# jakubbober/discrete-curvature-rewiring

Hardware: AMD Instinct MI355X
Metric: SDRF iterations/sec (higher is better)
Workload: dtype f64; 1 GPU; S100k: preferential-attachment graph N=100000 m=10 E=999900 (PCG64 seed 12345), Balanced Forman curvature, full recompute every iteration, remove_edges=True, tau=163.0, removal_bound=0.95; parallelism=single GPU

## Files before the change

### discrete-curvature-rewiring_amd/csrc/dcr_sdrf.hip

```cpp
#include <cstdlib>
#include "dcr_internal.h"
#include <cstdio>

namespace dcr {

struct RowView {
    const int2 *rowinfo;
    const int32_t *col;
    const int32_t *slot_row;
};

__device__ __host__ inline double bfc_formula(int d1, int d2, int T, int s1, int s2, int gamma) {
    int dmax = d1 > d2 ? d1 : d2, dmin = d1 < d2 ? d1 : d2;
    double r = 2.0 / (double)d1;
    r = r + 2.0 / (double)d2;
    r = r - 2.0;
    r = r + (double)(2 * (int64_t)T) / (double)dmax;
    r = r + (double)T / (double)dmin;
    if (s1 == 0 || s2 == 0) return r;
    double q = 1.0 / (double)gamma;
    q = q / (double)dmax;
    q = q * (double)(s1 + s2);
    return r + q;
}
// ... 21 lines not shown
            cv[q] = ok[q] ? curv[s] : 0.0;
        }
#pragma unroll
        for (int q = 0; q < 4; ++q) ru[q] = ok[q] ? g.rowinfo[u[q]] : make_int2(0, 0);
#pragma unroll
        for (int q = 0; q < 4; ++q) {
            const int64_t s = s0 + q * stride;
            if (!ok[q] || (int)(s - ru[q].x) >= ru[q].y || v[q] <= u[q]) continue;
            body((int)s, u[q], v[q], cv[q], acc...);
        }
    }
}

__global__ void __launch_bounds__(256) k_argext_edges(RowView g, int64_t cap_total, const double *curv, int want_max,
                                                       int excl_u, int excl_v, const DevResult *res, Ext *partial) {
    __shared__ double shv[4];
    __shared__ int shs[4];
    if (excl_u == -2) {
        excl_u = res->cand_i;
        excl_v = res->cand_j;
    }
    double best_v = 0.0;
    int best_s = -1;
    walk_edge_slots(
        g, cap_total, curv,
        [=](int s, int u, int v, double cv, double &bv, int &bs) {
            if (u == excl_u && v == excl_v) return;
            ext_take(bv, bs, cv, s, want_max);
        },
        best_v, best_s);
    ext_block_reduce(best_v, best_s, want_max, shv, shs);
    if (threadIdx.x == 0) partial[blockIdx.x] = ext_make(best_v, best_s);
}

__global__ void __launch_bounds__(256) k_argext_edges_both(RowView g, int64_t cap_total, const double *curv, Ext *part_min, Ext *part_max,
                                                            unsigned *clear_words, int64_t n_clear_words, DevResult *res) {
    __shared__ double shv[4];
    __shared__ int shs[4];
    for (int64_t i = (int64_t)blockIdx.x * blockDim.x + threadIdx.x; i < n_clear_words; i += (int64_t)gridDim.x * blockDim.x) clear_words[i] = 0u;
    if (n_clear_words > 0 && blockIdx.x == 0 && threadIdx.x == 0) res->touched_n = 0;
    double lo_v = 0.0, hi_v = 0.0;
    int lo_s = -1, hi_s = -1;
    walk_edge_slots(
        g, cap_total, curv,
        [](int s, int, int, double cv, double &lv, int &ls, double &hv, int &hs) {
            ext_take(lv, ls, cv, s, 0);
            ext_take(hv, hs, cv, s, 1);
        },
        lo_v, lo_s, hi_v, hi_s);
    ext_block_reduce(lo_v, lo_s, 0, shv, shs);
    if (threadIdx.x == 0) part_min[blockIdx.x] = ext_make(lo_v, lo_s);
    __syncthreads();
    ext_block_reduce(hi_v, hi_s, 1, shv, shs);
    if (threadIdx.x == 0) part_max[blockIdx.x] = ext_make(hi_v, hi_s);
}

__device__ inline void reduce_partials(const Ext *partial, int nparts, int want_max, double &best_v, int &best_s) {
    __shared__ double shv[16];
    __shared__ int shs[16];
    best_v = 0.0;
    best_s = -1;
    for (int i = threadIdx.x; i < nparts; i += blockDim.x) {
        const Ext e = partial[i];
        ext_take(best_v, best_s, e.val, e.slot, want_max);
    }
    ext_block_reduce(best_v, best_s, want_max, shv, shs);
}

__device__ inline void argext_final_body(const RowView &g, const Ext *partial, int nparts, int want_max, DevResult *res) {
    double best_v;
    int best_s;
    reduce_partials(partial, nparts, want_max, best_v, best_s);
    if (threadIdx.x == 0) {
        res->ext_val = best_v;
        res->ext_slot = best_s;
        const int eu = best_s >= 0 ? g.slot_row[best_s] : -1, ev = best_s >= 0 ? g.col[best_s] : -1;
        res->ext_u = eu;
        res->ext_v = ev;
        res->ext_du = best_s >= 0 ? g.rowinfo[eu].y : 0;
        res->ext_dv = best_s >= 0 ? g.rowinfo[ev].y : 0;
    }
}

__global__ void __launch_bounds__(1024) k_argext_final(RowView g, const Ext *partial, int nparts, int want_max,
                                                        DevResult *res) {
    argext_final_body(g, partial, nparts, want_max, res);
}

__global__ void __launch_bounds__(256) k_argmax_array(const double *a, int64_t n, const DevResult *res, Ext *partial) {
    __shared__ double shv[4];
    __shared__ int shs[4];
    if (res) n = res->n_cand;
    double best_v = 0.0;
    int best_s = -1;
    for (int64_t i = (int64_t)blockIdx.x * blockDim.x + threadIdx.x; i < n; i += (int64_t)gridDim.x * blockDim.x) {
        ext_take(best_v, best_s, a[i], (int)i, 1);
    }
    ext_block_reduce(best_v, best_s, 1, shv, shs);
    if (threadIdx.x == 0) partial[blockIdx.x] = ext_make(best_v, best_s);
}

__global__ void __launch_bounds__(256) k_argmax_final(const Ext *partial, int nparts, DevResult *res) {
    double best_v;
    int best_s;
    reduce_partials(partial, nparts, 1, best_v, best_s);
    if (threadIdx.x == 0) res->imp_argmax = best_s;
}

__device__ inline void store_candidate(DevResult *res, const int32_t *ci, const int32_t *cj, int64_t idx) {
    const int32_t a = ci[idx], b = cj[idx];
    res->cand_i = a < b ? a : b;
    res->cand_j = a < b ? b : a;
}

constexpr unsigned T_EMPTY = 0xFFFFFFFFu;

__device__ inline unsigned g_hash(unsigned key, unsigned mask) { return (key * 0x9E3779B1u >> 7) & mask; }

__device__ inline int g_find(const int32_t *keys, unsigned mask, int key) {
    unsigned h = g_hash((unsigned)key, mask);
    while (true) {
        const int e = keys[h];
        if (e == key) return (int)h;
        if ((unsigned)e == T_EMPTY) return -1;
        h = (h + 1) & mask;
    }
}

__device__ inline void g_find4(const int32_t *keys, unsigned mask, const int (&key)[4], const bool (&valid)[4], int (&out)[4]) {
    unsigned h[4];
    int e[4];
#pragma unroll
    for (int q = 0; q < 4; ++q) {
        h[q] = g_hash((unsigned)key[q], mask);
        e[q] = valid[q] ? keys[h[q]] : (int)T_EMPTY;
    }
#pragma unroll
    for (int q = 0; q < 4; ++q) {
        out[q] = -1;
        if (!valid[q]) continue;
        while (true) {
            if (e[q] == key[q]) { out[q] = (int)h[q]; break; }
            if ((unsigned)e[q] == T_EMPTY) break;
            h[q] = (h[q] + 1) & mask;
            e[q] = keys[h[q]];
        }
    }
}

struct ImpBuf {
    int32_t *keys, *posx, *posy;
    int32_t *c1, *c2;
    int32_t *clsx, *clsy;
    double *impb, *impc;
    int32_t *rowcount, *rowoff;
    uint32_t *adjbits;
    ImpStats *st;
};

__global__ void __launch_bounds__(256) k_imp_insert(RowView g, ImpBuf B, int x, int y, unsigned mask, const Ext *amax_parts, int amax_n,
                                                     DevResult *res) {
    const int nblocks = (int)gridDim.x - (amax_parts ? 1 : 0);
    if ((int)blockIdx.x == nblocks) {
        argext_final_body(g, amax_parts, amax_n, 1, res);
        return;
    }
    const int2 rx = g.rowinfo[x], ry = g.rowinfo[y];
    const int total = rx.y + ry.y;
    for (int t = blockIdx.x * blockDim.x + threadIdx.x; t < total; t += nblocks * blockDim.x) {
        const bool isx = t < rx.y;
        const int p = isx ? t : t - rx.y;
        const int k = g.col[(isx ? rx.x : ry.x) + p];
        if (isx) {
            B.c1[p] = 0;
            B.clsx[p] = k == y ? 2 : 0;
        } else {
            B.c2[p] = 0;
            B.clsy[p] = k == x ? 2 : 0;
            if (k == x) B.st->pos_x_in_y = p;
        }
        if (k == (isx ? y : x)) continue;
        unsigned h = g_hash((unsigned)k, mask);
        while (true) {
            const unsigned old = atomicCAS((unsigned *)&B.keys[h], T_EMPTY, (unsigned)k);
            if (old == T_EMPTY || old == (unsigned)k) break;
            h = (h + 1) & mask;
        }
        if (isx) B.posx[h] = p;
        else B.posy[h] = p;
    }
    if (blockIdx.x == 0 && threadIdx.x == 0) {
        B.st->x = x;
        B.st->y = y;
        B.st->dx = rx.y;
        B.st->dy = ry.y;
        B.st->table_mask = (int)mask;
        B.st->T = 0;
        B.st->deg_min_is_one = (rx.y < ry.y ? rx.y : ry.y) == 1;
        B.st->done_rows = 0;
        B.st->done_draw = 0;
    }
}

__global__ void __launch_bounds__(256) k_imp_clear(ImpBuf B, int64_t ts) {
    const int64_t tid = (int64_t)blockIdx.x * blockDim.x + threadIdx.x, nth = (int64_t)gridDim.x * blockDim.x;
    for (int64_t i = tid; i < ts; i += nth) {
        B.keys[i] = -1;
        B.posx[i] = -1;
        B.posy[i] = -1;
    }
    if (tid == 0) B.st->pos_x_in_y = -1;
}

struct Mx {
    int m, c, s;
};

__device__ inline Mx mx_join(Mx a, Mx b) {
    Mx r;
    if (a.m == b.m) {
        r.m = a.m;
        r.c = a.c + b.c;
        r.s = a.s > b.s ? a.s : b.s;
    } else if (a.m > b.m) {
        r.m = a.m;
        r.c = a.c;
        r.s = a.s > b.m ? a.s : b.m;
    } else {
        r.m = b.m;
        r.c = b.c;
        r.s = b.s > a.m ? b.s : a.m;
    }
    return r;
}

__device__ inline Mx mx_add(Mx a, int v) {
    Mx b;
    b.m = v;
    b.c = 1;
    b.s = -1;
    return mx_join(a, b);
}

__device__ inline void block_stats(const int32_t *c, int n, int *cnt_pos, Mx *mx, int *shi) {
    int pos = 0;
    Mx m;
    m.m = -1;
    m.c = 0;
    m.s = -1;
    for (int i = threadIdx.x; i < n; i += blockDim.x) {
        const int v = c[i];
        pos += v > 0;
        m = mx_add(m, v);
    }
    for (int off = 32; off > 0; off >>= 1) {
        pos += __shfl_xor(pos, off);
        Mx o;
        o.m = __shfl_xor(m.m, off);
        o.c = __shfl_xor(m.c, off);
        o.s = __shfl_xor(m.s, off);
        m = mx_join(m, o);
    }
    const int lane = threadIdx.x & 63, wid = threadIdx.x >> 6, nw = blockDim.x >> 6;
    __syncthreads();
    if (lane == 0) {
        shi[wid * 4 + 0] = pos;
        shi[wid * 4 + 1] = m.m;
        shi[wid * 4 + 2] = m.c;
        shi[wid * 4 + 3] = m.s;
    }
    __syncthreads();
    pos = 0;
    m.m = -1;
    m.c = 0;
    m.s = -1;
    for (int w = 0; w < nw; ++w) {
        pos += shi[w * 4];
        Mx o;
        o.m = shi[w * 4 + 1];
        o.c = shi[w * 4 + 2];
        o.s = shi[w * 4 + 3];
        m = mx_join(m, o);
    }
    *cnt_pos = pos;
    *mx = m;
}

__device__ inline void imp_close_stats(ImpBuf B, int curv_type, int *shi) {
    ImpStats *st = B.st;
    const int dx = st->dx, dy = st->dy;
    int s1, s2;
    Mx m1, m2;
    block_stats(B.c1, dx, &s1, &m1, shi);
    block_stats(B.c2, dy, &s2, &m2, shi);
    int T = 0;
    for (int a = threadIdx.x; a < dx; a += blockDim.x) T += B.clsx[a] == 1;
    for (int off = 32; off > 0; off >>= 1) T += __shfl_xor(T, off);
    __syncthreads();
    if ((threadIdx.x & 63) == 0) shi[threadIdx.x >> 6] = T;
    __syncthreads();
    if (threadIdx.x == 0) {
        T = 0;
        for (int w = 0; w < (int)(blockDim.x >> 6); ++w) T += shi[w];
        st->T = T;
        st->s1 = s1;
        st->s2 = s2;
        st->max1 = m1.m < 0 ? 0 : m1.m;
        st->cnt1 = m1.c;
        st->sec1 = m1.s < 0 ? 0 : m1.s;
        st->max2 = m2.m < 0 ? 0 : m2.m;
        st->cnt2 = m2.c;
        st->sec2 = m2.s < 0 ? 0 : m2.s;
        const int gam = st->max1 > st->max2 ? st->max1 : st->max2;
        double before;
        switch (curv_type) {
            case DCR_CURV_1D: before = (double)(4 - dx - dy); break;
            case DCR_CURV_AUGMENTED: before = (double)(4 - dx - dy + 3 * T); break;
            case DCR_CURV_HAANTJES: before = (double)T; break;
            default: before = bfc_value(dx, dy, T, s1, s2, gam);
        }
        st->before = before;
    }
    __syncthreads();
}

__global__ void __launch_bounds__(256) k_imp_bc(RowView g, ImpBuf B, int x, int y, unsigned mask, int curv_type) {
    __shared__ int dec_sh, maxadj_sh;
    const ImpStats st = *B.st;
    const int lane = threadIdx.x & 63;
    const int wv = blockIdx.x;
    if (wv >= st.dx + st.dy) return;
    const bool isB = wv < st.dy;
    const int p = isB ? wv : wv - st.dy;
    const int cls = isB ? B.clsy[p] : B.clsx[p];
    double *out = isB ? B.impb : B.impc;
    if (cls != 0) {
        if (threadIdx.x == 0) out[p] = 0.0;
        return;
    }
    if (curv_type != DCR_CURV_BFC) {
        const double d = curv_type == DCR_CURV_1D ? -1.0 : curv_type == DCR_CURV_AUGMENTED ? 2.0 : 1.0;
        if (threadIdx.x == 0) out[p] = d;
        return;
    }
    if (threadIdx.x == 0) {
        dec_sh = 0;
        maxadj_sh = 0;
    }
    __syncthreads();
    const int2 rown = g.rowinfo[isB ? y : x];
    const int node = g.col[rown.x + p];
    const int2 rn = g.rowinfo[node];
    const int32_t *cnt_other = isB ? B.c1 : B.c2;
    const int max_other = isB ? st.max1 : st.max2;
    int n_dec0 = 0, n_maxadj = 0;
    for (int base = 0; base < rn.y; base += 4 * 256) {
        int w[4], h[4];
        bool in[4];
#pragma unroll
        for (int q = 0; q < 4; ++q) {
            const int t = base + 256 * q + (int)threadIdx.x;
            in[q] = t < rn.y;
            w[q] = in[q] ? g.col[rn.x + t] : -1;
        }
        g_find4(B.keys, mask, w, in, h);
#pragma unroll
        for (int q = 0; q < 4; ++q) {
            bool dec0 = false, mxa = false;
            if (h[q] >= 0) {
                const int px = B.posx[h[q]], py = B.posy[h[q]];
                const bool other_only = isB ? (px >= 0 && py < 0) : (py >= 0 && px < 0);
                if (other_only) {
                    const int c = cnt_other[isB ? px : py];
                    dec0 = (c == 1);
                    mxa = (c == max_other);
                }
            }
            n_dec0 += __popcll(__ballot(dec0));
            n_maxadj += __popcll(__ballot(mxa));
        }
    }
    if (lane == 0) {
        if (n_dec0) atomicAdd(&dec_sh, n_dec0);
        if (n_maxadj) atomicAdd(&maxadj_sh, n_maxadj);
    }
    __syncthreads();
    n_dec0 = dec_sh;
    n_maxadj = maxadj_sh;
    if (threadIdx.x != 0) return;
    int s1, s2, m1, m2, d1, d2;
    if (isB) {
        const int cb = B.c2[p];
        s1 = st.s1 - n_dec0;
        m1 = (st.max1 > 0 && n_maxadj == st.cnt1) ? st.max1 - 1 : st.max1;
        s2 = st.s2 - (cb > 0);
        m2 = (cb == st.max2 && st.cnt2 == 1) ? st.sec2 : st.max2;
        d1 = st.dx + 1;
        d2 = st.dy;
    } else {
        const int ca = B.c1[p];
        s2 = st.s2 - n_dec0;
        m2 = (st.max2 > 0 && n_maxadj == st.cnt2) ? st.max2 - 1 : st.max2;
        s1 = st.s1 - (ca > 0);
        m1 = (ca == st.max1 && st.cnt1 == 1) ? st.sec1 : st.max1;
        d1 = st.dx;
        d2 = st.dy + 1;
    }
    const double after = bfc_value(d1, d2, st.T + 1, s1, s2, m1 > m2 ? m1 : m2);
    out[p] = after - st.before;
}

__global__ void __launch_bounds__(256) k_imp_rows_count(RowView g, ImpBuf B, int x, int y, unsigned mask, int words, int curv_type,
                                                         DevResult *res) {
    extern __shared__ uint32_t bits[];
    __shared__ int cnt_sh, c1_sh;
    __shared__ int shi[16 * 4];
    ImpStats *stp = B.st;
    const int dx = stp->dx, dy = stp->dy;
    const int pos_x_in_y = stp->pos_x_in_y;
    const int a = blockIdx.x;
    const int2 rx = g.rowinfo[x], ry = g.rowinfo[y];
    const int i = a < dx ? g.col[rx.x + a] : x;
    for (int w = threadIdx.x; w < words; w += blockDim.x) bits[w] = 0u;
    int cls = 3, b_i = -1;
    if (i == y) {
        cls = 2;
        b_i = dy;
    } else if (i == x) {
        b_i = pos_x_in_y;
    } else {
        const int h = g_find(B.keys, mask, i);
        if (h >= 0) b_i = B.posy[h];
        if (a < dx) cls = b_i >= 0 ? 1 : 0;
    }
    if (threadIdx.x == 0) {
        cnt_sh = 0;
        c1_sh = 0;
        if (a < dx) __hip_atomic_store(&B.clsx[a], cls, __ATOMIC_RELAXED, __HIP_MEMORY_SCOPE_AGENT);
    }
    __syncthreads();
    const bool counting = curv_type == DCR_CURV_BFC && cls == 0;
    const int2 ri = g.rowinfo[i];
    int c = 0;
    for (int base = 0; base < ri.y; base += 4 * 256) {
        int w[4], h[4];
        bool in[4];
#pragma unroll
        for (int q = 0; q < 4; ++q) {
            const int t = base + 256 * q + (int)threadIdx.x;
            in[q] = t < ri.y;
            w[q] = in[q] ? g.col[ri.x + t] : -1;
            in[q] = in[q] && w[q] != x && w[q] != y;
        }
        g_find4(B.keys, mask, w, in, h);
#pragma unroll
        for (int q = 0; q < 4; ++q) {
            int b = -1;
            if (w[q] == y && base + 256 * q + (int)threadIdx.x < ri.y) b = dy;
            else if (w[q] == x && base + 256 * q + (int)threadIdx.x < ri.y) b = pos_x_in_y;
            else if (in[q] && h[q] >= 0) {
                b = B.posy[h[q]];
                if (counting && b >= 0 && B.posx[h[q]] < 0) {
                    ++c;
                    atomicAdd(&B.c2[b], 1);
                }
            }
            if (b >= 0) atomicOr(&bits[b >> 5], 1u << (b & 31));
        }
    }
    if (threadIdx.x == 0 && b_i >= 0) atomicOr(&bits[b_i >> 5], 1u << (b_i & 31));
    for (int b = a + (int)threadIdx.x * (int)gridDim.x; b < dy; b += (int)blockDim.x * (int)gridDim.x) {
        const int k = g.col[ry.x + b];
        if (k != x) {
            const int h = g_find(B.keys, mask, k);
            B.clsy[b] = (h >= 0 && B.posx[h] >= 0) ? 1 : 0;
        }
    }
    for (int off = 32; off > 0; off >>= 1) c += __shfl_xor(c, off);
    if ((threadIdx.x & 63) == 0 && c) atomicAdd(&c1_sh, c);
    __syncthreads();
    int adm = 0;
    const int nb = dy + 1;
    for (int w = threadIdx.x; w < words; w += blockDim.x) {
        uint32_t v = bits[w];
        const int lo = w * 32;
        const uint32_t live = (nb - lo >= 32) ? 0xFFFFFFFFu : ((1u << (nb - lo)) - 1u);
        adm += __popc(~v & live);
        B.adjbits[(size_t)a * words + w] = v;
    }
    for (int off = 32; off > 0; off >>= 1) adm += __shfl_xor(adm, off);
    if ((threadIdx.x & 63) == 0 && adm) atomicAdd(&cnt_sh, adm);
    __syncthreads();
    if (threadIdx.x == 0) {
        __hip_atomic_store(&B.rowcount[a], cnt_sh, __ATOMIC_RELAXED, __HIP_MEMORY_SCOPE_AGENT);
        if (a < dx) __hip_atomic_store(&B.c1[a], counting ? c1_sh : 0, __ATOMIC_RELAXED, __HIP_MEMORY_SCOPE_AGENT);
    }
    if (!last_arriver(&stp->done_rows, (int)gridDim.x)) return;
    __builtin_amdgcn_fence(__ATOMIC_ACQUIRE, "agent");
    imp_close_stats(B, curv_type, shi);
    const int rows = (int)gridDim.x;
    __shared__ int wsum[4];
    __shared__ int carry_sh;
    if (threadIdx.x == 0) carry_sh = 0;
    __syncthreads();
    const int lane = threadIdx.x & 63, wid = threadIdx.x >> 6;
    for (int base = 0; base < rows; base += 256) {
        const int r = base + (int)threadIdx.x;
        const int v = r < rows ? __hip_atomic_load(&B.rowcount[r], __ATOMIC_RELAXED, __HIP_MEMORY_SCOPE_AGENT) : 0;
        int incl = v;
        for (int off = 1; off < 64; off <<= 1) {
            const int t = __shfl_up(incl, off);
            if (lane >= off) incl += t;
        }
        if (lane == 63) wsum[wid] = incl;
        __syncthreads();
        int woff = 0;
        for (int w = 0; w < wid; ++w) woff += wsum[w];
        const int carry = carry_sh;
        if (r < rows) B.rowoff[r] = carry + woff + incl - v;
        __syncthreads();
        if (threadIdx.x == 255) carry_sh = carry + woff + incl;
        __syncthreads();
    }
    if (threadIdx.x == 0) res->n_cand = carry_sh;
}

__global__ void __launch_bounds__(256) k_imp_emit(RowView g, ImpBuf B, int x, int y, int words, int curv_type,
                                                   double *out, int32_t *ci, int32_t *cj, int64_t ts) {
    __shared__ int wsum[4];
    __shared__ int carry_sh;
    const ImpStats st = *B.st;
    const int a = blockIdx.x;
    for (int64_t i = (int64_t)a * 256 + threadIdx.x; i < ts; i += (int64_t)gridDim.x * 256) {
        B.keys[i] = -1;
        B.posx[i] = -1;
        B.posy[i] = -1;
    }
    if (a == 0 && threadIdx.x == 0) B.st->pos_x_in_y = -1;
    if (B.rowcount[a] == 0) return;
    const int2 rx = g.rowinfo[x], ry = g.rowinfo[y];
    const int i = a < st.dx ? g.col[rx.x + a] : x;
    const int cls_a = a < st.dx ? B.clsx[a] : 3;
    const int c1a = (a < st.dx && cls_a == 0) ? B.c1[a] : 0;
    const int gam = st.max1 > st.max2 ? st.max1 : st.max2;
    const int nb = st.dy + 1;
    const int64_t row_base = B.rowoff[a];
    if (threadIdx.x == 0) carry_sh = 0;
    __syncthreads();
    const int lane = threadIdx.x & 63, wid = threadIdx.x >> 6;
    const unsigned long long lt = lane == 0 ? 0ull : (~0ull >> (64 - lane));
    for (int bbase = 0; bbase < nb; bbase += 256) {
        const int b = bbase + threadIdx.x;
        bool ok = false;
        if (b < nb) ok = ((B.adjbits[(size_t)a * words + (b >> 5)] >> (b & 31)) & 1u) == 0u;
        const unsigned long long m = __ballot(ok);
        if (lane == 0) wsum[wid] = __popcll(m);
        __syncthreads();
        int woff = 0;
        for (int q = 0; q < wid; ++q) woff += wsum[q];
        const int carry = carry_sh;
        if (ok) {
            const int64_t o = row_base + carry + woff + __popcll(m & lt);
            const int j = b < st.dy ? g.col[ry.x + b] : y;
            double val;
            if (a == st.dx) {
                val = B.impb[b];
            } else if (b == st.dy) {
                val = B.impc[a];
            } else if (curv_type == DCR_CURV_BFC && cls_a == 0 && B.clsy[b] == 0) {
                const int c2b = B.c2[b];
                const int mm = (c1a + 1 > c2b + 1 ? c1a + 1 : c2b + 1);
                const double after = bfc_value(st.dx, st.dy, st.T, st.s1 + (c1a == 0), st.s2 + (c2b == 0),
                                               mm > gam ? mm : gam);
                val = after - st.before;
            } else {
                val = 0.0;
            }
            out[o] = val;
            ci[o] = i < j ? i : j;
            cj[o] = i < j ? j : i;
        }
        __syncthreads();
        if (threadIdx.x == 0) carry_sh = carry + wsum[0] + wsum[1] + wsum[2] + wsum[3];
        __syncthreads();
    }
}

__global__ void k_pick_candidate(const int32_t *ci, const int32_t *cj, int64_t index, DevResult *res) {
    store_candidate(res, ci, cj, index);
    res->draw_status = 0;
}

constexpr int DRAW_BLOCKS = 256;

__global__ void k_draw_from_argmax(const int32_t *ci, const int32_t *cj, DevResult *res) {
    const int64_t n = res->n_cand, idx = res->imp_argmax;
    if (n <= 0) {
        res->draw_status = 2;
        res->draw_idx = -1;
        return;
    }
    if (idx < 0 || idx >= n) {
        res->draw_status = 1;
        res->draw_idx = -1;
        return;
    }
    store_candidate(res, ci, cj, idx);
    res->draw_idx = idx;
    res->draw_status = 0;
}

__device__ inline void draw_segment(int64_t n, int b, int t, int64_t &t0, int64_t &t1) {
    const int64_t L = (n + DRAW_BLOCKS - 1) / DRAW_BLOCKS, l = (L + 255) / 256;
    const int64_t b0 = (int64_t)b * L, bend = b0 + L < n ? b0 + L : n;
    t0 = b0 + (int64_t)t * l;
    t1 = t0 + l < bend ? t0 + l : bend;
}

__device__ inline double draw_segment_sum(const double *__restrict__ imp, int64_t n, double tau, int b, int t) {
    int64_t t0, t1;
    draw_segment(n, b, t, t0, t1);
    double s = 0.0;
    for (int64_t k = t0; k < t1; ++k) s += exp(imp[k] * tau);
    return s;
}

__device__ void draw_block_sum(const double *__restrict__ imp, const DevResult *res, double tau, double *__restrict__ bsum) {
    __shared__ double red[256];
    red[threadIdx.x] = draw_segment_sum(imp, res->n_cand, tau, (int)blockIdx.x, (int)threadIdx.x);
    __syncthreads();
    for (int st = 128; st > 0; st >>= 1) {
        if ((int)threadIdx.x < st) red[threadIdx.x] += red[threadIdx.x + st];
        __syncthreads();
    }
    if (threadIdx.x == 0) __hip_atomic_store(&bsum[blockIdx.x], red[0], __ATOMIC_RELAXED, __HIP_MEMORY_SCOPE_AGENT);
}

__device__ void draw_pick_block(const double *__restrict__ imp, const int32_t *__restrict__ ci, const int32_t *__restrict__ cj,
                                DevResult *res, double tau, double u, const double *bsum, double margin_scale) {
    __shared__ double pre[256];
    __shared__ int found;
    const int t = threadIdx.x;
    const int64_t n = res->n_cand;
    if (n <= 0) {
        if (t == 0) {
            res->draw_status = 2;
            res->draw_idx = -1;
        }
        return;
    }
    pre[t] = __hip_atomic_load(&bsum[t], __ATOMIC_RELAXED, __HIP_MEMORY_SCOPE_AGENT);
    __syncthreads();
    if (t == 0) {
        double a = 0.0;
        for (int k = 0; k < DRAW_BLOCKS; ++k) {
            a += pre[k];
            pre[k] = a;
        }
        found = DRAW_BLOCKS;
    }
    __syncthreads();
    const double total = pre[DRAW_BLOCKS - 1];
    const double T = u * total;
    const bool fine = total > 1e-250 && total < 1e300;
    if (fine && pre[t] > T) atomicMin(&found, t);
    __syncthreads();
    const int bs = found;
    if (!fine || bs >= DRAW_BLOCKS) {
        if (t == 0) {
            res->draw_status = 1;
            res->draw_idx = -1;
            res->draw_total = total;
        }
        return;
    }
    const double base = bs == 0 ? 0.0 : pre[bs - 1];
    __syncthreads();
    pre[t] = draw_segment_sum(imp, n, tau, bs, t);
    __syncthreads();
    if (t == 0) {
        const double margin = (double)(n + 1024) * 0x1p-51 * total * margin_scale;
        double run = base;
        int64_t idx = -1;
        double below = 0.0, above = 0.0;
        for (int k = 0; k < 256 && idx < 0; ++k) {
            if (run + pre[k] > T) {
                int64_t s0, s1;
                draw_segment(n, bs, k, s0, s1);
                for (int64_t q = s0; q < s1; ++q) {
                    const double prev = run;
                    run += exp(imp[q] * tau);
                    if (run > T) {
                        idx = q;
                        below = T - prev;
                        above = run - T;
                        break;
                    }
                }
                break;
            }
            run += pre[k];
        }
        const bool ok = idx >= 0 && above > margin && (idx == 0 || below > margin);
        res->draw_total = total;
        res->draw_gap = idx >= 0 ? (above < below || idx == 0 ? above : below) / total : 0.0;
        res->draw_idx = ok ? idx : -1;
        res->draw_status = ok ? 0 : 1;
        if (ok) store_candidate(res, ci, cj, idx);
    }
}

__global__ void __launch_bounds__(256) k_draw_partial(const double *__restrict__ imp, const int32_t *__restrict__ ci,
                                                       const int32_t *__restrict__ cj, DevResult *res, double tau, double u,
                                                       double *bsum, double margin_scale, ImpStats *st) {
    draw_block_sum(imp, res, tau, bsum);
    if (!last_arriver(&st->done_draw, (int)gridDim.x)) return;
    draw_pick_block(imp, ci, cj, res, tau, u, bsum, margin_scale);
}

struct SdrfScratch {
    ImpBuf imp{};
    int64_t table_cap = 0;
    int64_t rows_cap = 0, bits_cap = 0;
    bool table_dirty = true;
    double *out = nullptr;
    int32_t *ci = nullptr, *cj = nullptr;
    int64_t out_cap = 0;
    double *out_h = nullptr;
    int32_t *ci_h = nullptr, *cj_h = nullptr;
    int64_t out_h_cap = 0, cand_h_cap = 0;
    int64_t n = 0;
    Ext *red_scratch = nullptr;
    double *draw_bsum = nullptr;
};

constexpr int ARGEXT_BLOCKS = 1024;

template <typename... T>
static void dev_release(T **...p) {
    ((*p ? (void)hipFree(*p) : (void)0), ...);
    ((*p = nullptr), ...);
}

template <typename... T>
static int regrow_group(int64_t *cap, int64_t need, int64_t next, T **...p) {
    if (need <= *cap) return DCR_OK;
    *cap = 0;
    dev_release(p...);
    int rc = DCR_OK;
    ((rc = rc == DCR_OK ? dev_alloc(p, next) : rc), ...);
    if (rc != DCR_OK) {
        dev_release(p...);
        return rc;
    }
    *cap = next;
    return DCR_OK;
}

template <typename T>
static int pinned_regrow(T **p, int64_t *cap, int64_t need) {
    if (need <= *cap) return DCR_OK;
    if (*p) (void)hipHostFree(*p);
    *p = nullptr;
    int64_t nc = need + need / 4 + 1024;
    void *q = nullptr;
    hipError_t e = hipHostMalloc(&q, (size_t)nc * sizeof(T), hipHostMallocDefault);
    if (e != hipSuccess) {
        set_error(std::string("hipHostMalloc: ") + hipGetErrorString(e));
        return DCR_ENOMEM;
    }
    *p = (T *)q;
    *cap = nc;
    return DCR_OK;
}

int sdrf_scratch_create(dcr_graph *g) {
    SdrfScratch *S = g->sdrf = new SdrfScratch();
    DCR_TRY(dev_alloc(&S->imp.st, 1));
    DCR_HIP(hipMemsetAsync(S->imp.st, 0xFF, sizeof(ImpStats), g->stream));
    DCR_TRY(dev_alloc(&S->draw_bsum, DRAW_BLOCKS));
    return DCR_OK;
}

void sdrf_scratch_destroy(dcr_graph *g) {
    SdrfScratch *S = g->sdrf;
    if (!S) return;
    ImpBuf &B = S->imp;
    dev_release(&B.keys, &B.posx, &B.posy, &B.c1, &B.c2, &B.clsx, &B.clsy, &B.impb, &B.impc, &B.rowcount, &B.rowoff, &B.adjbits, &B.st,
                &S->out, &S->ci, &S->cj, &S->red_scratch, &S->draw_bsum);
    if (S->out_h) (void)hipHostFree(S->out_h);
    if (S->ci_h) (void)hipHostFree(S->ci_h);
    if (S->cj_h) (void)hipHostFree(S->cj_h);
    delete S;
    g->sdrf = nullptr;
}

static int red_scratch_of(dcr_graph *g, Ext **out) {
    SdrfScratch &S = *g->sdrf;
    if (!S.red_scratch) DCR_TRY(dev_alloc(&S.red_scratch, ARGEXT_BLOCKS));
    *out = S.red_scratch;
    return DCR_OK;
}

static inline int nparts_threads(int nparts) { return nparts > 1024 ? 1024 : nparts > 256 ? 512 : 256; }

static inline unsigned argext_blocks(int64_t cap_total) {
    const int64_t blocks = (cap_total + 255) / 256;
    return (unsigned)(blocks > ARGEXT_BLOCKS ? ARGEXT_BLOCKS : blocks < 1 ? 1 : blocks);
}

int launch_argext(dcr_graph *g, int want_max, int excl_u, int excl_v, hipStream_t st) {
    if (!st) st = g->stream;
    g->amax_valid = false;
    Ext *partial = nullptr;
    DCR_TRY(red_scratch_of(g, &partial));
    RowView vw{g->rowinfo, g->col, g->slot_row};
    const unsigned blocks = argext_blocks(g->cap_total);
    hipLaunchKernelGGL(k_argext_edges, dim3(blocks), dim3(256), 0, st, vw, g->cap_total, g->curv, want_max, excl_u, excl_v, g->dres,
                       partial);
    hipLaunchKernelGGL(k_argext_final, dim3(1), dim3(nparts_threads((int)blocks)), 0, st, vw, (const Ext *)partial, (int)blocks,
                       want_max, g->dres);
    DCR_HIP(hipGetLastError());
    return DCR_OK;
}

int launch_argext_both(dcr_graph *g, hipStream_t st, bool clear_dirty) {
    if (!st) st = g->stream;
    if (!g->ext_part) {
        Ext *p = nullptr;
        DCR_TRY(dev_alloc(&p, 2 * EXT_PART_BLOCKS));
        g->ext_part = p;
    }
    RowView vw{g->rowinfo, g->col, g->slot_row};
    const unsigned blocks = argext_blocks(g->cap_total);
    hipLaunchKernelGGL(k_argext_edges_both, dim3(blocks), dim3(256), 0, st, vw, g->cap_total, g->curv, (Ext *)g->ext_part,
                       (Ext *)g->ext_part + EXT_PART_BLOCKS, reinterpret_cast<unsigned *>(g->dirty),
                       clear_dirty ? (int64_t)(g->n + 3) / 4 : (int64_t)0, g->dres);
    DCR_HIP(hipGetLastError());
    g->ext_part_n = (int)blocks;
    g->ext_part_valid = true;
    return DCR_OK;
}

int launch_argext_from_parts(dcr_graph *g, int want_max, hipStream_t st) {
    if (!st) st = g->stream;
    g->amax_valid = false;
    RowView vw{g->rowinfo, g->col, g->slot_row};
    const Ext *parts = (const Ext *)g->ext_part + (want_max ? EXT_PART_BLOCKS : 0);
    hipLaunchKernelGGL(k_argext_final, dim3(1), dim3(nparts_threads(g->ext_part_n)), 0, st, vw, parts, g->ext_part_n, want_max, g->dres);
    DCR_HIP(hipGetLastError());
    return DCR_OK;
}

}

using namespace dcr;

static int imp_enqueue(dcr_graph *g, int32_t x, int32_t y, int curv_type, int64_t *upper_out, bool amax_from_parts = false) {
    int dx, dy;
    if (g->am_valid && g->am_x == x && g->am_y == y) {
        dx = g->am_dx;
        dy = g->am_dy;
    } else {
        int2 rxy[2];
        DCR_HIP(hipMemcpyAsync(&rxy[0], g->rowinfo + x, sizeof(int2), hipMemcpyDeviceToHost, g->stream));
        DCR_HIP(hipMemcpyAsync(&rxy[1], g->rowinfo + y, sizeof(int2), hipMemcpyDeviceToHost, g->stream));
        DCR_HIP(hipStreamSynchronize(g->stream));
        dx = rxy[0].y;
        dy = rxy[1].y;
    }
    const int64_t keys = (int64_t)dx + dy;
    int64_t ts = 64;
    while (ts < 4 * keys) ts <<= 1;
    const unsigned mask = (unsigned)(ts - 1);
    const int rows = dx + 1;
    const int words = (dy + 1 + 31) / 32;
    if ((size_t)words * 4 > 150 * 1024) DCR_FAIL(DCR_ECAPACITY, "deg(y) too large for the candidate bitmap");
    const int64_t upper = (int64_t)(dx + 1) * (dy + 1);
    if (upper > INT32_MAX) DCR_FAIL(DCR_ECAPACITY, "more than 2^31 candidate pairs");

    SdrfScratch &S = *g->sdrf;
    ImpBuf &B = S.imp;
    if (ts > S.table_cap) S.table_dirty = true;
    DCR_TRY(regrow_group(&S.table_cap, ts, ts, &B.keys, &B.posx, &B.posy));
    const int64_t rows_need = (int64_t)(dx > dy ? dx : dy) + 2;
    DCR_TRY(regrow_group(&S.rows_cap, rows_need, 2 * rows_need + 64, &B.c1, &B.c2, &B.rowcount, &B.rowoff, &B.clsx, &B.clsy, &B.impb,
                         &B.impc));
    if ((int64_t)rows * words > S.bits_cap) DCR_TRY(dev_regrow(&B.adjbits, &S.bits_cap, 2 * (int64_t)rows * words));
    DCR_TRY(regrow_group(&S.out_cap, upper, 2 * upper + 1024, &S.out, &S.ci, &S.cj));
    RowView vw{g->rowinfo, g->col, g->slot_row};

    if (S.table_dirty) {
        const unsigned blocks = (unsigned)((S.table_cap + 255) / 256 > 1024 ? 1024 : (S.table_cap + 255) / 256);
        hipLaunchKernelGGL(k_imp_clear, dim3(blocks ? blocks : 1), dim3(256), 0, g->stream, B, S.table_cap);
    }
    S.table_dirty = true;
    const int gi = (dx + dy + 255) / 256 > 0 ? (dx + dy + 255) / 256 : 1;
    const Ext *amax_parts = amax_from_parts ? (const Ext *)g->ext_part + EXT_PART_BLOCKS : nullptr;
    hipLaunchKernelGGL(k_imp_insert, dim3(gi + (amax_parts ? 1 : 0)), dim3(256), 0, g->stream, vw, B, x, y, mask, amax_parts,
                       amax_parts ? g->ext_part_n : 0, g->dres);
    hipLaunchKernelGGL(k_imp_rows_count, dim3(rows), dim3(256), (size_t)words * 4, g->stream, vw, B, x, y, mask, words, curv_type,
                       g->dres);
    if (dx + dy > 0)
        hipLaunchKernelGGL(k_imp_bc, dim3(dx + dy), dim3(256), 0, g->stream, vw, B, x, y, mask, curv_type);
    hipLaunchKernelGGL(k_imp_emit, dim3(rows), dim3(256), 0, g->stream, vw, B, x, y, words, curv_type, S.out, S.ci, S.cj, ts);
    S.table_dirty = false;
    DCR_HIP(hipGetLastError());
    *upper_out = upper;
    return DCR_OK;
}

static int check_edge_args(const dcr_graph *g, int32_t x, int32_t y, int curv_type) {
    if (x < 0 || y < 0 || x >= g->n || y >= g->n || x == y) DCR_FAIL(DCR_EINVAL, "bad node ids");
    if (curv_type < DCR_CURV_BFC || curv_type > DCR_CURV_HAANTJES) DCR_FAIL(DCR_EINVAL, "unknown curvature type");
    return DCR_OK;
}

static int pick_candidate(dcr_graph *g, int64_t cand_index) {
    if (!g) DCR_FAIL(DCR_EINVAL, "null graph");
    if (cand_index < 0 || cand_index >= g->sdrf->n) DCR_FAIL(DCR_EINVAL, "candidate index out of range");
    DCR_HIP(hipSetDevice(g->device));
    hipLaunchKernelGGL(k_pick_candidate, dim3(1), dim3(1), 0, g->stream, g->sdrf->ci, g->sdrf->cj, cand_index, g->dres);
    return DCR_OK;
}

static void fill_added(const dcr_graph *g, int32_t out_added[2]) {
    if (!out_added) return;
    out_added[0] = g->hres->cand_i;
    out_added[1] = g->hres->cand_j;
}

extern "C" {

int dcr_argext(dcr_graph *g, int want_max, int32_t excl_u, int32_t excl_v, int32_t *out_u, int32_t *out_v,
               double *out_val) {
    if (!g) DCR_FAIL(DCR_EINVAL, "null graph");
    if (!g->curv_valid) DCR_FAIL(DCR_ESTATE, "dcr_argext needs a curvature pass first");
    DCR_HIP(hipSetDevice(g->device));
    if (excl_u > excl_v) {
        int32_t t = excl_u;
        excl_u = excl_v;
        excl_v = t;
    }
    DCR_TRY(launch_argext(g, want_max, excl_u, excl_v));
    DCR_TRY(sync_result(g));
    if (g->hres->ext_slot < 0) DCR_FAIL(DCR_ENOTFOUND, "graph has no (eligible) edges");
    if (out_u) *out_u = g->hres->ext_u;
    if (out_v) *out_v = g->hres->ext_v;
    if (out_val) *out_val = g->hres->ext_val;
    return DCR_OK;
}

int dcr_improvements(dcr_graph *g, int32_t x, int32_t y, int curv_type, int want_candidates, int64_t *n_out,
                     const double **out_improvement, const int32_t **out_ci, const int32_t **out_cj) {
    if (!g || !n_out) DCR_FAIL(DCR_EINVAL, "null argument");
    DCR_TRY(check_edge_args(g, x, y, curv_type));
    DCR_HIP(hipSetDevice(g->device));
    SdrfScratch &S = *g->sdrf;
    int64_t upper = 0;
    DCR_TRY(imp_enqueue(g, x, y, curv_type, &upper));
    if (upper > 0 && out_improvement) {
        DCR_TRY(pinned_regrow(&S.out_h, &S.out_h_cap, upper));
        DCR_HIP(hipMemcpyAsync(S.out_h, S.out, sizeof(double) * (size_t)upper, hipMemcpyDeviceToHost, g->stream));
    }
    if (upper > 0 && want_candidates) {
        if (upper > S.cand_h_cap) {
            int64_t c1 = S.cand_h_cap, c2 = S.cand_h_cap;
            DCR_TRY(pinned_regrow(&S.ci_h, &c1, upper));
            DCR_TRY(pinned_regrow(&S.cj_h, &c2, upper));
            S.cand_h_cap = c1 < c2 ? c1 : c2;
        }
        DCR_HIP(hipMemcpyAsync(S.ci_h, S.ci, sizeof(int32_t) * (size_t)upper, hipMemcpyDeviceToHost, g->stream));
        DCR_HIP(hipMemcpyAsync(S.cj_h, S.cj, sizeof(int32_t) * (size_t)upper, hipMemcpyDeviceToHost, g->stream));
    }
    DCR_TRY(sync_result(g));
    const int64_t n = g->hres->n_cand;
    if (n < 0 || n > upper) DCR_FAIL(DCR_ESTATE, "candidate count outside its bound");
    S.n = n;
    *n_out = n;
    if (g->curv_valid && n > 0) {
        if (g->ext_part_valid) DCR_TRY(launch_argext_from_parts(g, 1));
        else DCR_TRY(launch_argext(g, 1, -1, -1));
        g->amax_valid = true;
    }
    if (out_improvement) *out_improvement = n > 0 ? S.out_h : nullptr;
    if (out_ci) *out_ci = (n > 0 && want_candidates) ? S.ci_h : nullptr;
    if (out_cj) *out_cj = (n > 0 && want_candidates) ? S.cj_h : nullptr;
    return DCR_OK;
}

int dcr_improvements_argmax(dcr_graph *g, int64_t *out_index) {
    if (!g || !out_index) DCR_FAIL(DCR_EINVAL, "null argument");
    const int64_t n = g->sdrf->n;
    if (n <= 0) DCR_FAIL(DCR_ESTATE, "no candidates from the last dcr_improvements call");
    DCR_HIP(hipSetDevice(g->device));
    Ext *partial = nullptr;
    DCR_TRY(red_scratch_of(g, &partial));
    const int64_t blocks = (n + 255) / 256 > ARGEXT_BLOCKS ? ARGEXT_BLOCKS : (n + 255) / 256;
    hipLaunchKernelGGL(k_argmax_array, dim3((unsigned)blocks), dim3(256), 0, g->stream, g->sdrf->out, n, (const DevResult *)nullptr,
                       partial);
    hipLaunchKernelGGL(k_argmax_final, dim3(1), dim3(256), 0, g->stream, (const Ext *)partial, (int)blocks, g->dres);
    DCR_HIP(hipGetLastError());
    DCR_TRY(sync_result(g));
    *out_index = g->hres->imp_argmax;
    return DCR_OK;
}

int dcr_candidate_at(dcr_graph *g, int64_t index, int32_t *out_i, int32_t *out_j) {
    if (!g || !out_i || !out_j) DCR_FAIL(DCR_EINVAL, "null argument");
    if (index < 0 || index >= g->sdrf->n) DCR_FAIL(DCR_EINVAL, "candidate index out of range");
    DCR_HIP(hipSetDevice(g->device));
    DCR_HIP(hipMemcpyAsync(out_i, g->sdrf->ci + index, sizeof(int32_t), hipMemcpyDeviceToHost, g->stream));
    DCR_HIP(hipMemcpyAsync(out_j, g->sdrf->cj + index, sizeof(int32_t), hipMemcpyDeviceToHost, g->stream));
    DCR_HIP(hipStreamSynchronize(g->stream));
    return DCR_OK;
}

}

struct TailCall {
    int32_t add_k, add_l;
    int do_remove;
    double bound;
    bool adding, have_amax;
    int edit_add, edit_rem;
};

struct TailPass {
    int curv_type, incremental;
    int32_t *out_u, *out_v;
    double *out_val;
};

static int tail_prepare(dcr_graph *g, int32_t add_k, int32_t add_l, int do_remove, double removal_bound, TailCall *tc) {
    if (!g) DCR_FAIL(DCR_EINVAL, "null graph");
    if (do_remove && !g->curv_valid) DCR_FAIL(DCR_ESTATE, "removal needs a curvature pass first");
    tc->adding = add_k >= 0 || add_k == -2;
    if (add_k >= 0) {
        if (add_l < 0 || add_k >= g->n || add_l >= g->n || add_k == add_l) DCR_FAIL(DCR_EINVAL, "bad edge to add");
        if (add_k > add_l) {
            int32_t t = add_k;
            add_k = add_l;
            add_l = t;
        }
    }
    tc->add_k = add_k;
    tc->add_l = add_l;
    tc->do_remove = do_remove;
    tc->bound = removal_bound;
    DCR_HIP(hipSetDevice(g->device));
    g->am_valid = false;
    tc->have_amax = g->amax_valid;
    g->amax_valid = false;
    tc->edit_add = g->pending_edits;
    tc->edit_rem = g->pending_edits + (tc->adding ? 1 : 0);
    g->pending_edits += (tc->adding ? 1 : 0) + (do_remove ? 1 : 0);
    return DCR_OK;
}
// ... 156 lines not shown
```

Baseline: 1209 iterations/sec.

## Fold boundary-candidate improvement kernel into emit using adjacency bitmap and neighbor descriptors

Removes the separate k_imp_bc kernel, which re-walked each neighbor's adjacency list through hash-table probes. Boundary candidates are now computed inside k_imp_emit: the x row counts adjacent bits per bitmap word, and the y column accumulates ballot counts while rows are emitted. The insert kernel also caches per-neighbor descriptors (node, row offset, degree, hash slot) so later kernels skip repeated hash lookups and rowinfo loads. Scans are restructured to use double-buffered shared sums instead of carry syncs, cutting one launch and several barriers but adding atomics and more complex indexing.

```diff
diff --git a/discrete-curvature-rewiring_amd/csrc/dcr_sdrf.hip b/discrete-curvature-rewiring_amd/csrc/dcr_sdrf.hip
--- a/discrete-curvature-rewiring_amd/csrc/dcr_sdrf.hip
+++ b/discrete-curvature-rewiring_amd/csrc/dcr_sdrf.hip
@@ -197,7 +197,7 @@
     int32_t *keys, *posx, *posy;
     int32_t *c1, *c2;
     int32_t *clsx, *clsy;
-    double *impb, *impc;
+    int4 *descx, *descy;
     int32_t *rowcount, *rowoff;
     uint32_t *adjbits;
     ImpStats *st;
@@ -216,6 +216,7 @@
         const bool isx = t < rx.y;
         const int p = isx ? t : t - rx.y;
         const int k = g.col[(isx ? rx.x : ry.x) + p];
+        const int2 rk = g.rowinfo[k];
         if (isx) {
             B.c1[p] = 0;
             B.clsx[p] = k == y ? 2 : 0;
@@ -224,15 +225,19 @@
             B.clsy[p] = k == x ? 2 : 0;
             if (k == x) B.st->pos_x_in_y = p;
         }
-        if (k == (isx ? y : x)) continue;
-        unsigned h = g_hash((unsigned)k, mask);
-        while (true) {
-            const unsigned old = atomicCAS((unsigned *)&B.keys[h], T_EMPTY, (unsigned)k);
-            if (old == T_EMPTY || old == (unsigned)k) break;
-            h = (h + 1) & mask;
-        }
-        if (isx) B.posx[h] = p;
-        else B.posy[h] = p;
+        int slot = -1;
+        if (k != (isx ? y : x)) {
+            unsigned h = g_hash((unsigned)k, mask);
+            while (true) {
+                const unsigned old = atomicCAS((unsigned *)&B.keys[h], T_EMPTY, (unsigned)k);
+                if (old == T_EMPTY || old == (unsigned)k) break;
+                h = (h + 1) & mask;
+            }
+            if (isx) B.posx[h] = p;
+            else B.posy[h] = p;
+            slot = (int)h;
+        }
+        (isx ? B.descx : B.descy)[p] = make_int4(k, rk.x, rk.y, slot);
     }
     if (blockIdx.x == 0 && threadIdx.x == 0) {
         B.st->x = x;
@@ -244,6 +249,7 @@
         B.st->deg_min_is_one = (rx.y < ry.y ? rx.y : ry.y) == 1;
         B.st->done_rows = 0;
         B.st->done_draw = 0;
+        B.descx[rx.y] = make_int4(x, rx.x, rx.y, -1);
     }
 }
 
@@ -369,114 +375,26 @@
     __syncthreads();
 }
 
-__global__ void __launch_bounds__(256) k_imp_bc(RowView g, ImpBuf B, int x, int y, unsigned mask, int curv_type) {
-    __shared__ int dec_sh, maxadj_sh;
-    const ImpStats st = *B.st;
-    const int lane = threadIdx.x & 63;
-    const int wv = blockIdx.x;
-    if (wv >= st.dx + st.dy) return;
-    const bool isB = wv < st.dy;
-    const int p = isB ? wv : wv - st.dy;
-    const int cls = isB ? B.clsy[p] : B.clsx[p];
-    double *out = isB ? B.impb : B.impc;
-    if (cls != 0) {
-        if (threadIdx.x == 0) out[p] = 0.0;
-        return;
-    }
-    if (curv_type != DCR_CURV_BFC) {
-        const double d = curv_type == DCR_CURV_1D ? -1.0 : curv_type == DCR_CURV_AUGMENTED ? 2.0 : 1.0;
-        if (threadIdx.x == 0) out[p] = d;
-        return;
-    }
-    if (threadIdx.x == 0) {
-        dec_sh = 0;
-        maxadj_sh = 0;
-    }
-    __syncthreads();
-    const int2 rown = g.rowinfo[isB ? y : x];
-    const int node = g.col[rown.x + p];
-    const int2 rn = g.rowinfo[node];
-    const int32_t *cnt_other = isB ? B.c1 : B.c2;
-    const int max_other = isB ? st.max1 : st.max2;
-    int n_dec0 = 0, n_maxadj = 0;
-    for (int base = 0; base < rn.y; base += 4 * 256) {
-        int w[4], h[4];
-        bool in[4];
-#pragma unroll
-        for (int q = 0; q < 4; ++q) {
-            const int t = base + 256 * q + (int)threadIdx.x;
-            in[q] = t < rn.y;
-            w[q] = in[q] ? g.col[rn.x + t] : -1;
-        }
-        g_find4(B.keys, mask, w, in, h);
-#pragma unroll
-        for (int q = 0; q < 4; ++q) {
-            bool dec0 = false, mxa = false;
-            if (h[q] >= 0) {
-                const int px = B.posx[h[q]], py = B.posy[h[q]];
-                const bool other_only = isB ? (px >= 0 && py < 0) : (py >= 0 && px < 0);
-                if (other_only) {
-                    const int c = cnt_other[isB ? px : py];
-                    dec0 = (c == 1);
-                    mxa = (c == max_other);
-                }
-            }
-            n_dec0 += __popcll(__ballot(dec0));
-            n_maxadj += __popcll(__ballot(mxa));
-        }
-    }
-    if (lane == 0) {
-        if (n_dec0) atomicAdd(&dec_sh, n_dec0);
-        if (n_maxadj) atomicAdd(&maxadj_sh, n_maxadj);
-    }
-    __syncthreads();
-    n_dec0 = dec_sh;
-    n_maxadj = maxadj_sh;
-    if (threadIdx.x != 0) return;
-    int s1, s2, m1, m2, d1, d2;
-    if (isB) {
-        const int cb = B.c2[p];
-        s1 = st.s1 - n_dec0;
-        m1 = (st.max1 > 0 && n_maxadj == st.cnt1) ? st.max1 - 1 : st.max1;
-        s2 = st.s2 - (cb > 0);
-        m2 = (cb == st.max2 && st.cnt2 == 1) ? st.sec2 : st.max2;
-        d1 = st.dx + 1;
-        d2 = st.dy;
-    } else {
-        const int ca = B.c1[p];
-        s2 = st.s2 - n_dec0;
-        m2 = (st.max2 > 0 && n_maxadj == st.cnt2) ? st.max2 - 1 : st.max2;
-        s1 = st.s1 - (ca > 0);
-        m1 = (ca == st.max1 && st.cnt1 == 1) ? st.sec1 : st.max1;
-        d1 = st.dx;
-        d2 = st.dy + 1;
-    }
-    const double after = bfc_value(d1, d2, st.T + 1, s1, s2, m1 > m2 ? m1 : m2);
-    out[p] = after - st.before;
-}
-
-__global__ void __launch_bounds__(256) k_imp_rows_count(RowView g, ImpBuf B, int x, int y, unsigned mask, int words, int curv_type,
-                                                         DevResult *res) {
+__global__ void __launch_bounds__(256) k_imp_rows_count(RowView g, ImpBuf B, int x, int y, int dy, unsigned mask, int words,
+                                                         int curv_type, DevResult *res) {
     extern __shared__ uint32_t bits[];
     __shared__ int cnt_sh, c1_sh;
     __shared__ int shi[16 * 4];
     ImpStats *stp = B.st;
-    const int dx = stp->dx, dy = stp->dy;
+    const int dx = (int)gridDim.x - 1;
+    const int a = blockIdx.x;
+    const int4 d = B.descx[a];
     const int pos_x_in_y = stp->pos_x_in_y;
-    const int a = blockIdx.x;
-    const int2 rx = g.rowinfo[x], ry = g.rowinfo[y];
-    const int i = a < dx ? g.col[rx.x + a] : x;
     for (int w = threadIdx.x; w < words; w += blockDim.x) bits[w] = 0u;
     int cls = 3, b_i = -1;
-    if (i == y) {
+    if (a == dx) {
+        b_i = pos_x_in_y;
+    } else if (d.w < 0) {
         cls = 2;
         b_i = dy;
-    } else if (i == x) {
-        b_i = pos_x_in_y;
     } else {
-        const int h = g_find(B.keys, mask, i);
-        if (h >= 0) b_i = B.posy[h];
-        if (a < dx) cls = b_i >= 0 ? 1 : 0;
+        b_i = B.posy[d.w];
+        cls = b_i >= 0 ? 1 : 0;
     }
     if (threadIdx.x == 0) {
         cnt_sh = 0;
@@ -485,7 +403,7 @@
     }
     __syncthreads();
     const bool counting = curv_type == DCR_CURV_BFC && cls == 0;
-    const int2 ri = g.rowinfo[i];
+    const int2 ri = make_int2(d.y, d.z);
     int c = 0;
     for (int base = 0; base < ri.y; base += 4 * 256) {
         int w[4], h[4];
@@ -515,11 +433,8 @@
     }
     if (threadIdx.x == 0 && b_i >= 0) atomicOr(&bits[b_i >> 5], 1u << (b_i & 31));
     for (int b = a + (int)threadIdx.x * (int)gridDim.x; b < dy; b += (int)blockDim.x * (int)gridDim.x) {
-        const int k = g.col[ry.x + b];
-        if (k != x) {
-            const int h = g_find(B.keys, mask, k);
-            B.clsy[b] = (h >= 0 && B.posx[h] >= 0) ? 1 : 0;
-        }
+        const int h = B.descy[b].w;
+        if (h >= 0) B.clsy[b] = B.posx[h] >= 0 ? 1 : 0;
     }
     for (int off = 32; off > 0; off >>= 1) c += __shfl_xor(c, off);
     if ((threadIdx.x & 63) == 0 && c) atomicAdd(&c1_sh, c);
@@ -544,36 +459,65 @@
     __builtin_amdgcn_fence(__ATOMIC_ACQUIRE, "agent");
     imp_close_stats(B, curv_type, shi);
     const int rows = (int)gridDim.x;
-    __shared__ int wsum[4];
-    __shared__ int carry_sh;
-    if (threadIdx.x == 0) carry_sh = 0;
-    __syncthreads();
+    __shared__ int wsum[2][4];
     const int lane = threadIdx.x & 63, wid = threadIdx.x >> 6;
-    for (int base = 0; base < rows; base += 256) {
-        const int r = base + (int)threadIdx.x;
-        const int v = r < rows ? __hip_atomic_load(&B.rowcount[r], __ATOMIC_RELAXED, __HIP_MEMORY_SCOPE_AGENT) : 0;
-        int incl = v;
+    int carry = 0;
+    for (int base = 0, par = 0; base < rows; base += 4 * 256, par ^= 1) {
+        const int r0 = base + 4 * (int)threadIdx.x;
+        int v[4];
+#pragma unroll
+        for (int q = 0; q < 4; ++q)
+            v[q] = r0 + q < rows ? __hip_atomic_load(&B.rowcount[r0 + q], __ATOMIC_RELAXED, __HIP_MEMORY_SCOPE_AGENT) : 0;
+        const int mine = v[0] + v[1] + v[2] + v[3];
+        int incl = mine;
         for (int off = 1; off < 64; off <<= 1) {
             const int t = __shfl_up(incl, off);
             if (lane >= off) incl += t;
         }
-        if (lane == 63) wsum[wid] = incl;
+        if (lane == 63) wsum[par][wid] = incl;
         __syncthreads();
-        int woff = 0;
-        for (int w = 0; w < wid; ++w) woff += wsum[w];
-        const int carry = carry_sh;
-        if (r < rows) B.rowoff[r] = carry + woff + incl - v;
-        __syncthreads();
-        if (threadIdx.x == 255) carry_sh = carry + woff + incl;
-        __syncthreads();
-    }
-    if (threadIdx.x == 0) res->n_cand = carry_sh;
-}
-
-__global__ void __launch_bounds__(256) k_imp_emit(RowView g, ImpBuf B, int x, int y, int words, int curv_type,
+        int woff = 0, all = 0;
+#pragma unroll
+        for (int w = 0; w < 4; ++w) {
+            const int s = wsum[par][w];
+            woff += w < wid ? s : 0;
+            all += s;
+        }
+        int o = carry + woff + incl - mine;
+#pragma unroll
+        for (int q = 0; q < 4; ++q) {
+            if (r0 + q < rows) B.rowoff[r0 + q] = o;
+            o += v[q];
+        }
+        carry += all;
+    }
+    if (threadIdx.x == 0) res->n_cand = carry;
+}
+
+__device__ inline double bfc_after_b(const ImpStats &st, int cb, int n_dec0, int n_maxadj) {
+    const int s1 = st.s1 - n_dec0;
+    const int m1 = (st.max1 > 0 && n_maxadj == st.cnt1) ? st.max1 - 1 : st.max1;
+    const int s2 = st.s2 - (cb > 0);
+    const int m2 = (cb == st.max2 && st.cnt2 == 1) ? st.sec2 : st.max2;
+    return bfc_value(st.dx + 1, st.dy, st.T + 1, s1, s2, m1 > m2 ? m1 : m2);
+}
+
+__device__ inline double bfc_after_c(const ImpStats &st, int ca, int n_dec0, int n_maxadj) {
+    const int s2 = st.s2 - n_dec0;
+    const int m2 = (st.max2 > 0 && n_maxadj == st.cnt2) ? st.max2 - 1 : st.max2;
+    const int s1 = st.s1 - (ca > 0);
+    const int m1 = (ca == st.max1 && st.cnt1 == 1) ? st.sec1 : st.max1;
+    return bfc_value(st.dx, st.dy + 1, st.T + 1, s1, s2, m1 > m2 ? m1 : m2);
+}
+
+__device__ inline double classical_bc(int curv_type) {
+    return curv_type == DCR_CURV_1D ? -1.0 : curv_type == DCR_CURV_AUGMENTED ? 2.0 : 1.0;
+}
+
+__global__ void __launch_bounds__(256) k_imp_emit(ImpBuf B, int x, int y, int dx, int dy, int words, int curv_type,
                                                    double *out, int32_t *ci, int32_t *cj, int64_t ts) {
-    __shared__ int wsum[4];
-    __shared__ int carry_sh;
+    __shared__ int wsum[2][4];
+    __shared__ int dec_sh[32], mxa_sh[32];
     const ImpStats st = *B.st;
     const int a = blockIdx.x;
     for (int64_t i = (int64_t)a * 256 + threadIdx.x; i < ts; i += (int64_t)gridDim.x * 256) {
@@ -582,53 +526,106 @@
         B.posy[i] = -1;
     }
     if (a == 0 && threadIdx.x == 0) B.st->pos_x_in_y = -1;
+    const int nb = dy + 1;
+    const bool bfc = curv_type == DCR_CURV_BFC;
+    const int lane = threadIdx.x & 63, wid = threadIdx.x >> 6;
+    if (a >= dx) {
+        const int wc = a - dx, lo = wc * 32;
+        const uint32_t *rowx = B.adjbits + (size_t)dx * words;
+        const uint32_t live = (nb - lo >= 32) ? 0xFFFFFFFFu : ((1u << (nb - lo)) - 1u);
+        const uint32_t adm = ~rowx[wc] & live;
+        if (adm == 0u) return;
+        if (threadIdx.x < 32) dec_sh[threadIdx.x] = mxa_sh[threadIdx.x] = 0;
+        int before = 0;
+        for (int w = threadIdx.x; w < wc; w += 256) before += __popc(~rowx[w]);
+        for (int off = 32; off > 0; off >>= 1) before += __shfl_xor(before, off);
+        if (lane == 0) wsum[0][wid] = before;
+        __syncthreads();
+        before = wsum[0][0] + wsum[0][1] + wsum[0][2] + wsum[0][3];
+        if (bfc) {
+            for (int r = threadIdx.x; r < dx; r += 256) {
+                const int c = B.c1[r];
+                if (B.clsx[r] != 0 || (c != 1 && c != st.max1)) continue;
+                uint32_t m = B.adjbits[(size_t)r * words + wc] & adm;
+                while (m) {
+                    const int bit = __ffs(m) - 1;
+                    m &= m - 1u;
+                    if (c == 1) atomicAdd(&dec_sh[bit], 1);
+                    if (c == st.max1) atomicAdd(&mxa_sh[bit], 1);
+                }
+            }
+            __syncthreads();
+        }
+        if (threadIdx.x < 32 && ((adm >> threadIdx.x) & 1u)) {
+            const int b = lo + (int)threadIdx.x;
+            const int64_t o = (int64_t)B.rowoff[dx] + before + __popc(adm & ((1u << threadIdx.x) - 1u));
+            const int j = b < dy ? B.descy[b].x : y;
+            out[o] = bfc ? bfc_after_b(st, B.c2[b], dec_sh[threadIdx.x], mxa_sh[threadIdx.x]) - st.before : classical_bc(curv_type);
+            ci[o] = x < j ? x : j;
+            cj[o] = x < j ? j : x;
+        }
+        return;
+    }
     if (B.rowcount[a] == 0) return;
-    const int2 rx = g.rowinfo[x], ry = g.rowinfo[y];
-    const int i = a < st.dx ? g.col[rx.x + a] : x;
-    const int cls_a = a < st.dx ? B.clsx[a] : 3;
-    const int c1a = (a < st.dx && cls_a == 0) ? B.c1[a] : 0;
+    const int i = B.descx[a].x;
+    const int cls_a = B.clsx[a];
+    const int c1a = cls_a == 0 ? B.c1[a] : 0;
     const int gam = st.max1 > st.max2 ? st.max1 : st.max2;
-    const int nb = st.dy + 1;
     const int64_t row_base = B.rowoff[a];
-    if (threadIdx.x == 0) carry_sh = 0;
-    __syncthreads();
-    const int lane = threadIdx.x & 63, wid = threadIdx.x >> 6;
+    const bool general = bfc && cls_a == 0;
     const unsigned long long lt = lane == 0 ? 0ull : (~0ull >> (64 - lane));
-    for (int bbase = 0; bbase < nb; bbase += 256) {
+    int carry = 0, n_dec0 = 0, n_maxadj = 0;
+    int64_t o_y = -1;
+    for (int bbase = 0, par = 0; bbase < nb; bbase += 256, par ^= 1) {
         const int b = bbase + threadIdx.x;
         bool ok = false;
         if (b < nb) ok = ((B.adjbits[(size_t)a * words + (b >> 5)] >> (b & 31)) & 1u) == 0u;
+        int clsyb = 3, c2b = 0;
+        if (general && b < dy) {
+            clsyb = B.clsy[b];
+            c2b = B.c2[b];
+        }
+        const bool adj = general && b < dy && !ok && clsyb == 0;
+        n_dec0 += __popcll(__ballot(adj && c2b == 1));
+        n_maxadj += __popcll(__ballot(adj && c2b == st.max2));
         const unsigned long long m = __ballot(ok);
-        if (lane == 0) wsum[wid] = __popcll(m);
+        if (lane == 0) wsum[par][wid] = __popcll(m);
         __syncthreads();
-        int woff = 0;
-        for (int q = 0; q < wid; ++q) woff += wsum[q];
-        const int carry = carry_sh;
+        int woff = 0, all = 0;
+#pragma unroll
+        for (int q = 0; q < 4; ++q) {
+            const int s = wsum[par][q];
+            woff += q < wid ? s : 0;
+            all += s;
+        }
         if (ok) {
             const int64_t o = row_base + carry + woff + __popcll(m & lt);
-            const int j = b < st.dy ? g.col[ry.x + b] : y;
-            double val;
-            if (a == st.dx) {
-                val = B.impb[b];
-            } else if (b == st.dy) {
-                val = B.impc[a];
-            } else if (curv_type == DCR_CURV_BFC && cls_a == 0 && B.clsy[b] == 0) {
-                const int c2b = B.c2[b];
+            const int j = b < dy ? B.descy[b].x : y;
+            if (b == dy) {
+                o_y = o;
+            } else if (general && clsyb == 0) {
                 const int mm = (c1a + 1 > c2b + 1 ? c1a + 1 : c2b + 1);
                 const double after = bfc_value(st.dx, st.dy, st.T, st.s1 + (c1a == 0), st.s2 + (c2b == 0),
                                                mm > gam ? mm : gam);
-                val = after - st.before;
+                out[o] = after - st.before;
             } else {
-                val = 0.0;
+                out[o] = 0.0;
             }
-            out[o] = val;
             ci[o] = i < j ? i : j;
             cj[o] = i < j ? j : i;
         }
-        __syncthreads();
-        if (threadIdx.x == 0) carry_sh = carry + wsum[0] + wsum[1] + wsum[2] + wsum[3];
-        __syncthreads();
-    }
+        carry += all;
+    }
+    __syncthreads();
+    if (threadIdx.x == 0) dec_sh[0] = mxa_sh[0] = 0;
+    __syncthreads();
+    if (lane == 0 && general) {
+        if (n_dec0) atomicAdd(&dec_sh[0], n_dec0);
+        if (n_maxadj) atomicAdd(&mxa_sh[0], n_maxadj);
+    }
+    __syncthreads();
+    if (o_y >= 0)
+        out[o_y] = cls_a != 0 ? 0.0 : bfc ? bfc_after_c(st, c1a, dec_sh[0], mxa_sh[0]) - st.before : classical_bc(curv_type);
 }
 
 __global__ void k_pick_candidate(const int32_t *ci, const int32_t *cj, int64_t index, DevResult *res) {
@@ -831,7 +828,7 @@
     SdrfScratch *S = g->sdrf;
     if (!S) return;
     ImpBuf &B = S->imp;
-    dev_release(&B.keys, &B.posx, &B.posy, &B.c1, &B.c2, &B.clsx, &B.clsy, &B.impb, &B.impc, &B.rowcount, &B.rowoff, &B.adjbits, &B.st,
+    dev_release(&B.keys, &B.posx, &B.posy, &B.c1, &B.c2, &B.clsx, &B.clsy, &B.descx, &B.descy, &B.rowcount, &B.rowoff, &B.adjbits, &B.st,
                 &S->out, &S->ci, &S->cj, &S->red_scratch, &S->draw_bsum);
     if (S->out_h) (void)hipHostFree(S->out_h);
     if (S->ci_h) (void)hipHostFree(S->ci_h);
@@ -929,8 +926,8 @@
     if (ts > S.table_cap) S.table_dirty = true;
     DCR_TRY(regrow_group(&S.table_cap, ts, ts, &B.keys, &B.posx, &B.posy));
     const int64_t rows_need = (int64_t)(dx > dy ? dx : dy) + 2;
-    DCR_TRY(regrow_group(&S.rows_cap, rows_need, 2 * rows_need + 64, &B.c1, &B.c2, &B.rowcount, &B.rowoff, &B.clsx, &B.clsy, &B.impb,
-                         &B.impc));
+    DCR_TRY(regrow_group(&S.rows_cap, rows_need, 2 * rows_need + 64, &B.c1, &B.c2, &B.rowcount, &B.rowoff, &B.clsx, &B.clsy, &B.descx,
+                         &B.descy));
     if ((int64_t)rows * words > S.bits_cap) DCR_TRY(dev_regrow(&B.adjbits, &S.bits_cap, 2 * (int64_t)rows * words));
     DCR_TRY(regrow_group(&S.out_cap, upper, 2 * upper + 1024, &S.out, &S.ci, &S.cj));
     RowView vw{g->rowinfo, g->col, g->slot_row};
@@ -944,11 +941,9 @@
     const Ext *amax_parts = amax_from_parts ? (const Ext *)g->ext_part + EXT_PART_BLOCKS : nullptr;
     hipLaunchKernelGGL(k_imp_insert, dim3(gi + (amax_parts ? 1 : 0)), dim3(256), 0, g->stream, vw, B, x, y, mask, amax_parts,
                        amax_parts ? g->ext_part_n : 0, g->dres);
-    hipLaunchKernelGGL(k_imp_rows_count, dim3(rows), dim3(256), (size_t)words * 4, g->stream, vw, B, x, y, mask, words, curv_type,
-                       g->dres);
-    if (dx + dy > 0)
-        hipLaunchKernelGGL(k_imp_bc, dim3(dx + dy), dim3(256), 0, g->stream, vw, B, x, y, mask, curv_type);
-    hipLaunchKernelGGL(k_imp_emit, dim3(rows), dim3(256), 0, g->stream, vw, B, x, y, words, curv_type, S.out, S.ci, S.cj, ts);
+    hipLaunchKernelGGL(k_imp_rows_count, dim3(rows), dim3(256), (size_t)words * 4, g->stream, vw, B, x, y, dy, mask, words,
+                       curv_type, g->dres);
+    hipLaunchKernelGGL(k_imp_emit, dim3(dx + words), dim3(256), 0, g->stream, B, x, y, dx, dy, words, curv_type, S.out, S.ci, S.cj, ts);
     S.table_dirty = false;
     DCR_HIP(hipGetLastError());
     *upper_out = upper;
```

Result: faster. 1227 iterations/sec (median of 6 runs) (+1.4%).
